# andi611/ZeroSpeech-TTS-without-T

Measured on AMD Instinct MI355X. Metric: mel-frames/sec (train_ae, seg_len=128, enc_size=1024), higher is better.
Workload: dtype bf16; 1 GPU; train_ae english hps seg_len=128 enc_size=1024 emb_size=1024 n_speakers=102 F=513, batch=256/GPU, dropout+Gumbel on, fwd+bwd+clip+Adam; global_batch=256, parallelism=dp1

## Files before the change

zerospeech-tts-without-t_amd/csrc/zs_gemm.hip:

```cpp
#include <stdlib.h>

#include <atomic>
#include <mutex>

#include "zs_common.h"

namespace {

constexpr int BM = 128, BN = 128, NT = 256;
constexpr int ROWB = 128;
constexpr int PITCH = 144;
constexpr int TILE_BYTES = BM * PITCH;

__device__ const uint4 zs_zero_line[8] = {};

__device__ __forceinline__ int xcd_remap(int bid, int nwg) {
  const int q = nwg >> 3, r = nwg & 7, xcd = bid & 7;
  return (xcd < r ? xcd * (q + 1) : r * (q + 1) + (xcd - r) * q) + (bid >> 3);
}

__device__ __forceinline__ int conv_src_row(int gather, int pad_mode, int stride, int pad_left, int T_in, int t,
                                            int j, bool& ok) {
  if (gather == 0) {
    int s = t * stride + j - pad_left;
// ... 1224 lines not shown
__device__ __forceinline__ void wgrad_tile_store(const ZsGemmWgrad& p, unsigned char* smem, f32x16 (&acc)[2][2], bool do_bias,
                                                 const float (&bsum)[LPT][EPS], const int (&lrow)[LPT], const int (&lseg)[LPT],
                                                 int split, int nsplit, int co0, int ci0, int tap, int cout_r, int cin_r, int wm, int wn,
                                                 int lane, int tid) {
  if (do_bias) {
    float* red = reinterpret_cast<float*>(smem);
#pragma unroll
    for (int i = 0; i < LPT; ++i)
#pragma unroll
      for (int e = 0; e < EPS; ++e) red[lrow[i] * 128 + lseg[i] * EPS + e] = bsum[i][e];
    __syncthreads();
    if (tid < 128) {
      float t = 0.f;
#pragma unroll 8
      for (int r = 0; r < WK; ++r) t += red[r * 128 + tid];
      float* bslab = (float*)p.workspace + (int64_t)nsplit * cout_r * p.taps * cin_r + (int64_t)split * cout_r;
      bslab[co0 + tid] = t;
    }
  }
  float* slab = (float*)p.workspace + (int64_t)split * cout_r * p.taps * cin_r;
  float* sC = reinterpret_cast<float*>(smem);
  __syncthreads();
#pragma unroll
  for (int mi = 0; mi < 2; ++mi)
#pragma unroll
    for (int ni = 0; ni < 2; ++ni)
#pragma unroll
      for (int r = 0; r < 16; ++r) {
        const int row = wm * 64 + mi * 32 + (r & 3) + 8 * (r >> 2) + 4 * (lane >> 5);
        const int col = wn * 64 + ni * 32 + (lane & 31);
        sC[row * CPITCH + col] = acc[mi][ni][r];
      }
  __syncthreads();
  const int cg = tid & 15, rr0 = tid >> 4;
#pragma unroll 1
  for (int it = 0; it < 8; ++it) {
    const int row = rr0 + 16 * it;
    const float4 x0 = *reinterpret_cast<const float4*>(sC + row * CPITCH + cg * 8);
    const float4 x1 = *reinterpret_cast<const float4*>(sC + row * CPITCH + cg * 8 + 4);
    float* d = slab + ((int64_t)(co0 + row) * p.taps + tap) * cin_r + ci0 + cg * 8;
    *reinterpret_cast<float4*>(d) = x0;
    *reinterpret_cast<float4*>(d + 4) = x1;
  }
}

template <typename T>
__global__ __launch_bounds__(NT, 2) void gemm_wgrad_kernel(const ZsGemmWgrad p, int ci_tiles, int rows_per_split,
                                                          int cout_r, int cin_r) {
  const Geom2 g2 = make_geom2(p.w_in, p.w_out, p.taps_h, p.T_in);
  constexpr int EPS = 16 / (int)sizeof(T);
  constexpr int SPR = 128 / EPS;
  constexpr int LPT = (WK * SPR) / NT;
  constexpr int PITCHW = WFrag<T>::PITCHW;
  constexpr int TILEW = WK * PITCHW;
  extern __shared__ __attribute__((aligned(16))) unsigned char smem[];
  unsigned char* sY = smem;
  unsigned char* sX = smem + 2 * TILEW;

  const int tid = threadIdx.x, lane = tid & 63, wave = tid >> 6;
  const int wm = wave >> 1, wn = wave & 1;
  const int per_co = p.taps * ci_tiles;
  const int tiles = ((cout_r / 128) * per_co);
  const int vid = xcd_remap(blockIdx.x, gridDim.x);
  const int split = vid / tiles, tile = vid - split * tiles;
  const int cot = tile / per_co;
  const int rem = tile - cot * per_co;
  const int tap = rem / ci_tiles, cit = rem - tap * ci_tiles;
  const int co0 = cot * 128, ci0 = cit * 128;
  const int M = p.B * p.T_out;
  const int nsplit = gridDim.x / tiles;
  const int mbeg = split * rows_per_split;
  const int mend = min(M, mbeg + rows_per_split);
  const T* __restrict__ dY = (const T*)p.dY;
  const T* __restrict__ X = (const T*)p.X;

  int lrow[LPT], lseg[LPT], lb[LPT], lt[LPT];
#pragma unroll
  for (int i = 0; i < LPT; ++i) {
    const int idx = tid + NT * i;
    lrow[i] = idx / SPR; lseg[i] = idx - lrow[i] * SPR;
    const int m = mbeg + lrow[i];
    lb[i] = m / p.T_out; lt[i] = m - lb[i] * p.T_out;
  }
  uint4 vy[LPT], vx[LPT];
  const bool do_bias = (p.db != nullptr) && tap == 0 && cit == 0;
  float bsum[LPT][EPS];
#pragma unroll
  for (int i = 0; i < LPT; ++i)
#pragma unroll
    for (int e = 0; e < EPS; ++e) bsum[i][e] = 0.f;
  auto gload = [&](int mb) {
#pragma unroll
    for (int i = 0; i < LPT; ++i) {
      const int m = mb + lrow[i];
      const int cy = co0 + lseg[i] * EPS, cx = ci0 + lseg[i] * EPS;
      vy[i] = make_uint4(0, 0, 0, 0); vx[i] = make_uint4(0, 0, 0, 0);
      if (m < mend) {
        if (cy < p.y_cols) vy[i] = *reinterpret_cast<const uint4*>(dY + (int64_t)m * p.ldy + cy);
        bool ok; const int s = conv_src_row_g(0, p.pad_mode, p.stride, p.pad_left, p.T_in, lt[i], tap, ok, g2);
        if (ok && cx < p.x_cols)
          vx[i] = *reinterpret_cast<const uint4*>(X + (int64_t)lb[i] * p.x_batch_stride + (int64_t)s * p.ldx + cx);
      }
      lt[i] += WK;
      while (lt[i] >= p.T_out) { lt[i] -= p.T_out; ++lb[i]; }
    }
  };
  auto swrite = [&](int buf) {
#pragma unroll
    for (int i = 0; i < LPT; ++i) {
      *reinterpret_cast<uint4*>(sY + buf * TILEW + lrow[i] * PITCHW + lseg[i] * 16) = vy[i];
      *reinterpret_cast<uint4*>(sX + buf * TILEW + lrow[i] * PITCHW + lseg[i] * 16) = vx[i];
      if (do_bias) {
        const uint32_t w4[4] = {vy[i].x, vy[i].y, vy[i].z, vy[i].w};
        if constexpr (sizeof(T) == 4) {
#pragma unroll
          for (int e = 0; e < 4; ++e) bsum[i][e] += __uint_as_float(w4[e]);
        } else {
#pragma unroll
          for (int e = 0; e < 4; ++e) {
            bsum[i][2 * e] += __uint_as_float(w4[e] << 16);
            bsum[i][2 * e + 1] += __uint_as_float(w4[e] & 0xffff0000u);
          }
        }
      }
    }
  };

  f32x16 acc[2][2];
#pragma unroll
  for (int i = 0; i < 2; ++i)
#pragma unroll
    for (int j = 0; j < 2; ++j)
#pragma unroll
      for (int r = 0; r < 16; ++r) acc[i][j][r] = 0.f;

  const int nchunks = (mend - mbeg + WK - 1) / WK;
  if (nchunks > 0) {
    gload(mbeg);
    swrite(0);
  }
  __syncthreads();
  for (int c = 0; c < nchunks; ++c) {
    const int buf = c & 1;
    if (c + 1 < nchunks) gload(mbeg + (c + 1) * WK);
    WFrag<T>::chunk(sY + buf * TILEW, sX + buf * TILEW, wm, wn, lane, acc);
    if (c + 1 < nchunks) swrite(buf ^ 1);
    __syncthreads();
  }

  wgrad_tile_store<LPT, EPS>(p, smem, acc, do_bias, bsum, lrow, lseg, split, nsplit, co0, ci0, tap, cout_r, cin_r, wm, wn, lane, tid);
}

#define ZS_DSRT(dst, addr, off) asm volatile("ds_read_b64_tr_b16 %0, %1 offset:" #off : "=v"(dst) : "v"(addr))
#define ZS_WP_READ_A(base)                                                                        \
  ZS_DSRT(ya00, sa0, base + 0);    ZS_DSRT(yb00, sa0, base + 512);  ZS_DSRT(ya01, sa1, base + 0);    ZS_DSRT(yb01, sa1, base + 512);  \
  ZS_DSRT(ya10, sa0, base + 2048); ZS_DSRT(yb10, sa0, base + 2560); ZS_DSRT(ya11, sa1, base + 2048); ZS_DSRT(yb11, sa1, base + 2560); \
  ZS_DSRT(ya20, sa0, base + 4096); ZS_DSRT(yb20, sa0, base + 4608); ZS_DSRT(ya21, sa1, base + 4096); ZS_DSRT(yb21, sa1, base + 4608); \
  ZS_DSRT(ya30, sa0, base + 6144); ZS_DSRT(yb30, sa0, base + 6656); ZS_DSRT(ya31, sa1, base + 6144); ZS_DSRT(yb31, sa1, base + 6656);
#define ZS_WP_READ_B(x, sbx)                                                                      \
  ZS_DSRT(x##a0, sbx, 0);    ZS_DSRT(x##b0, sbx, 512);  ZS_DSRT(x##a1, sbx, 2048); ZS_DSRT(x##b1, sbx, 2560); \
  ZS_DSRT(x##a2, sbx, 4096); ZS_DSRT(x##b2, sbx, 4608); ZS_DSRT(x##a3, sbx, 6144); ZS_DSRT(x##b3, sbx, 6656);
#define ZS_WP_MMA(alo, ahi, blo, bhi, c)                                                          \
  c = __builtin_amdgcn_mfma_f32_32x32x16_bf16(__builtin_bit_cast(bf16x8, make_uint4(alo.x, alo.y, ahi.x, ahi.y)), \
                                               __builtin_bit_cast(bf16x8, make_uint4(blo.x, blo.y, bhi.x, bhi.y)), c, 0, 0, 0)
#define ZS_WP_DMA(cond, src, dst)                                                                 \
  __builtin_amdgcn_sched_barrier(0);                                                              \
  if (cond) __builtin_amdgcn_global_load_lds((gptr_t)(src), (lptr_t)(dst), 16, 0, 0);             \
  __builtin_amdgcn_sched_barrier(0);
#define ZS_WP_QUAD(c0, c1, x, cond, src0, dst0, src1, dst1)                                        \
  __builtin_amdgcn_s_setprio(1);                                                                  \
  ZS_WP_MMA(ya00, yb00, x##a0, x##b0, c0); ZS_WP_MMA(ya01, yb01, x##a0, x##b0, c1);               \
  ZS_WP_DMA(cond, src0, dst0)                                                                     \
  ZS_WP_MMA(ya10, yb10, x##a1, x##b1, c0); ZS_WP_MMA(ya11, yb11, x##a1, x##b1, c1); ZS_WP_MMA(ya20, yb20, x##a2, x##b2, c0); \
  ZS_WP_DMA(cond, src1, dst1)                                                                     \
  ZS_WP_MMA(ya21, yb21, x##a2, x##b2, c1); ZS_WP_MMA(ya30, yb30, x##a3, x##b3, c0); ZS_WP_MMA(ya31, yb31, x##a3, x##b3, c1); \
  __builtin_amdgcn_s_setprio(0);

__global__ __launch_bounds__(PNT, 2) void gemm_wgrad_p8_kernel(const ZsGemmWgrad p, int ci_tiles, int rows_per_split,
                                                              int cout_r, int cin_r) {
  const Geom2 g2 = make_geom2(p.w_in, p.w_out, p.taps_h, p.T_in);
  typedef bf16_t T;
  extern __shared__ __attribute__((aligned(16))) unsigned char smem[];
  typedef __attribute__((address_space(1))) const void* gptr_t;
  typedef __attribute__((address_space(3))) void* lptr_t;
  const int tid = threadIdx.x, lane = tid & 63, wave = __builtin_amdgcn_readfirstlane(tid >> 6);
  const int wr = wave >> 2, wc = wave & 3;
  const int per_co = p.taps * ci_tiles;
  const int tiles = (cout_r / 256) * per_co;
  const int vid = xcd_remap(blockIdx.x, gridDim.x);
  const int split = vid / tiles, tile = vid - split * tiles;
  const int cot = tile / per_co;
  const int rem = tile - cot * per_co;
  const int tap = rem / ci_tiles, cit = rem - tap * ci_tiles;
  const int co0 = cot * 256, ci0 = cit * 256;
  const int M = p.B * p.T_out;
  const int nsplit = gridDim.x / tiles;
  const int mbeg = split * rows_per_split;
  const int mend = min(M, mbeg + rows_per_split);
  const int nk = (mend - mbeg + 63) / 64;
  const T* __restrict__ dY = (const T*)p.dY;
  const T* __restrict__ X = (const T*)p.X;
  const T* zline = reinterpret_cast<const T*>(zs_zero_line);

  const int lrow = lane >> 3, slot = lane & 7;
  const int k0 = (wave & 3) * 16 + lrow, k1 = k0 + 8;
  const int cbl = wave >> 2;
  const int sg0 = slot ^ (((k0 >> 1) & 1) << 2), sg1 = slot ^ (((k1 >> 1) & 1) << 2);
  const int yc0 = co0 + cbl * 64 + sg0 * 8, yc1 = co0 + cbl * 64 + sg1 * 8;
  const int xc0 = ci0 + cbl * 64 + sg0 * 8, xc1 = ci0 + cbl * 64 + sg1 * 8;
  auto y_ptr = [&](int m, int col) -> const T* {
    return (m < mend && col < p.y_cols) ? dY + (int64_t)m * p.ldy + col : zline;
  };
  auto x_row = [&](int m, bool& ok) -> const T* {
    ok = false;
    if (m >= mend) return zline;
    const int b = m / p.T_out, t = m - b * p.T_out;
    const int srow = conv_src_row_g(0, p.pad_mode, p.stride, p.pad_left, p.T_in, t, tap, ok, g2);
    return X + (int64_t)b * p.x_batch_stride + (int64_t)srow * p.ldx;
  };

  unsigned char* const ldsA = smem + wave * 2048;
  unsigned char* const ldsB = smem + 32768 + wave * 2048;

  f32x16 c000, c001, c010, c011, c100, c101, c110, c111;
#pragma unroll
  for (int r = 0; r < 16; ++r) { c000[r] = 0.f; c001[r] = 0.f; c010[r] = 0.f; c011[r] = 0.f; c100[r] = 0.f; c101[r] = 0.f; c110[r] = 0.f; c111[r] = 0.f; }

  const int gi = lane >> 4, q = (lane >> 2) & 3, pp = lane & 3;
  const int sw = ((q >> 1) & 1) << 2;
  const int segl = 2 * (gi & 1) + (pp >> 1);
  const unsigned lds0 = (unsigned)(uintptr_t)(__attribute__((address_space(3))) unsigned char*)smem;
  const unsigned rowoff = (unsigned)((8 * (gi >> 1) + q) * 128 + (pp & 1) * 8);
  const unsigned a_l0 = lds0 + (unsigned)(wr * 2 * 64 * 128) + rowoff + (unsigned)(((0 + segl) ^ sw) * 16);
  const unsigned a_l1 = lds0 + (unsigned)(wr * 2 * 64 * 128) + rowoff + (unsigned)(((4 + segl) ^ sw) * 16);
  const unsigned b_l0 = lds0 + 32768u + (unsigned)(wc * 64 * 128) + rowoff + (unsigned)(((0 + segl) ^ sw) * 16);
  const unsigned b_l1 = lds0 + 32768u + (unsigned)(wc * 64 * 128) + rowoff + (unsigned)(((4 + segl) ^ sw) * 16);
  const int grp1 = wr;

  const bool do_bias = (p.db != nullptr) && tap == 0 && cit == 0;
  const int tg = tid & 255, seg16 = tg & 15, kr0 = tg >> 4;
  const unsigned bias_addr = lds0 + (unsigned)(((wr * 2 + (seg16 >> 3)) * 64 + kr0) * 128 + (((seg16 & 7) ^ (((kr0 >> 1) & 1) << 2)) * 16));
  float bsum[8];
#pragma unroll
  for (int e = 0; e < 8; ++e) bsum[e] = 0.f;

  {
    __builtin_amdgcn_global_load_lds((gptr_t)y_ptr(mbeg + k0, yc0), (lptr_t)(ldsA), 16, 0, 0);
    __builtin_amdgcn_global_load_lds((gptr_t)y_ptr(mbeg + k1, yc1), (lptr_t)(ldsA + 1024), 16, 0, 0);
    __builtin_amdgcn_global_load_lds((gptr_t)y_ptr(mbeg + k0, yc0 + 128), (lptr_t)(ldsA + 16384), 16, 0, 0);
    __builtin_amdgcn_global_load_lds((gptr_t)y_ptr(mbeg + k1, yc1 + 128), (lptr_t)(ldsA + 16384 + 1024), 16, 0, 0);
#pragma unroll
    for (int tt = 0; tt < 2; ++tt) {
      if (tt < nk) {
        bool ok0, ok1;
        const T* r0 = x_row(mbeg + tt * 64 + k0, ok0);
        const T* r1 = x_row(mbeg + tt * 64 + k1, ok1);
        unsigned char* d = ldsB + tt * PSTAGE;
        __builtin_amdgcn_global_load_lds((gptr_t)((ok0 && xc0 < p.x_cols) ? r0 + xc0 : zline), (lptr_t)(d), 16, 0, 0);
        __builtin_amdgcn_global_load_lds((gptr_t)((ok1 && xc1 < p.x_cols) ? r1 + xc1 : zline), (lptr_t)(d + 1024), 16, 0, 0);
        __builtin_amdgcn_global_load_lds((gptr_t)((ok0 && xc0 + 128 < p.x_cols) ? r0 + xc0 + 128 : zline), (lptr_t)(d + 16384), 16, 0, 0);
        __builtin_amdgcn_global_load_lds((gptr_t)((ok1 && xc1 + 128 < p.x_cols) ? r1 + xc1 + 128 : zline), (lptr_t)(d + 16384 + 1024), 16, 0, 0);
      }
    }
    if (nk > 1) asm volatile("s_waitcnt vmcnt(4)" ::: "memory");
    else asm volatile("s_waitcnt vmcnt(0)" ::: "memory");
  }
  __builtin_amdgcn_s_barrier();
  if (grp1) __builtin_amdgcn_s_barrier();

  uint2 ya00, yb00, ya01, yb01, ya10, yb10, ya11, yb11, ya20, yb20, ya21, yb21, ya30, yb30, ya31, yb31;
  uint2 f0a0, f0b0, f0a1, f0b1, f0a2, f0b2, f0a3, f0b3;
  uint2 f1a0, f1b0, f1a1, f1b1, f1a2, f1b2, f1a3, f1b3;
  for (int kt = 0; kt < nk; ++kt) {
    const int st = kt & 1;
    const unsigned so = (unsigned)(st * PSTAGE);
    const unsigned sa0 = a_l0 + so, sa1 = a_l1 + so, sb0 = b_l0 + so, sb1 = b_l1 + so;
    const bool has_a = kt + 1 < nk, has_b = kt + 2 < nk;
    unsigned char* const dA = ldsA + (st ^ 1) * PSTAGE;
    unsigned char* const dB = ldsB + st * PSTAGE;
    const int ma = mbeg + (kt + 1) * 64, mb = mbeg + (kt + 2) * 64;
    ZS_WP_READ_A(0)
    ZS_WP_READ_B(f0, sb0)
    const T* s0 = y_ptr(ma + k0, yc0);
    const T* s1 = y_ptr(ma + k1, yc1);
    asm volatile("s_waitcnt lgkmcnt(0)" ::: "memory");
    __builtin_amdgcn_s_barrier();
    __builtin_amdgcn_sched_barrier(0);
    ZS_WP_QUAD(c000, c001, f0, has_a, s0, dA, s1, dA + 1024)
    __builtin_amdgcn_s_barrier();
    __builtin_amdgcn_sched_barrier(0);
    ZS_WP_READ_B(f1, sb1)
    s0 = y_ptr(ma + k0, yc0 + 128);
    s1 = y_ptr(ma + k1, yc1 + 128);
    if (do_bias) {
      u32x4_t v0, v1, v2, v3;
      const unsigned ba = bias_addr + so;
      ZS_DSR(v0, ba, 0); ZS_DSR(v1, ba, 2048); ZS_DSR(v2, ba, 4096); ZS_DSR(v3, ba, 6144);
      asm volatile("s_waitcnt lgkmcnt(0)" ::: "memory");
      const unsigned w[16] = {v0.x, v0.y, v0.z, v0.w, v1.x, v1.y, v1.z, v1.w, v2.x, v2.y, v2.z, v2.w, v3.x, v3.y, v3.z, v3.w};
#pragma unroll
      for (int i = 0; i < 16; ++i) {
        bsum[2 * (i & 3)] += __uint_as_float(w[i] << 16);
        bsum[2 * (i & 3) + 1] += __uint_as_float(w[i] & 0xffff0000u);
      }
    }
    asm volatile("s_waitcnt lgkmcnt(0)" ::: "memory");
    __builtin_amdgcn_s_barrier();
    __builtin_amdgcn_sched_barrier(0);
    ZS_WP_QUAD(c010, c011, f1, has_a, s0, dA + 16384, s1, dA + 16384 + 1024)
    __builtin_amdgcn_s_barrier();
    __builtin_amdgcn_sched_barrier(0);
    ZS_WP_READ_A(8192)
    bool ok0, ok1;
    const T* r0 = x_row(mb + k0, ok0);
    const T* r1 = x_row(mb + k1, ok1);
    s0 = (ok0 && xc0 < p.x_cols) ? r0 + xc0 : zline;
    s1 = (ok1 && xc1 < p.x_cols) ? r1 + xc1 : zline;
    asm volatile("s_waitcnt lgkmcnt(0)" ::: "memory");
    __builtin_amdgcn_s_barrier();
    __builtin_amdgcn_sched_barrier(0);
    ZS_WP_QUAD(c110, c111, f1, has_b, s0, dB, s1, dB + 1024)
    __builtin_amdgcn_s_barrier();
    __builtin_amdgcn_sched_barrier(0);
    s0 = (ok0 && xc0 + 128 < p.x_cols) ? r0 + xc0 + 128 : zline;
    s1 = (ok1 && xc1 + 128 < p.x_cols) ? r1 + xc1 + 128 : zline;
    if (grp1) {
      if (has_b) asm volatile("s_waitcnt vmcnt(2)" ::: "memory");
      else asm volatile("s_waitcnt vmcnt(0)" ::: "memory");
    }
    __builtin_amdgcn_s_barrier();
    __builtin_amdgcn_sched_barrier(0);
    ZS_WP_QUAD(c100, c101, f0, has_b, s0, dB + 16384, s1, dB + 16384 + 1024)
    if (!grp1) {
      if (has_b) asm volatile("s_waitcnt vmcnt(4)" ::: "memory");
      else asm volatile("s_waitcnt vmcnt(0)" ::: "memory");
    }
    __builtin_amdgcn_s_barrier();
    __builtin_amdgcn_sched_barrier(0);
  }
  if (!grp1) __builtin_amdgcn_s_barrier();
  asm volatile("s_waitcnt vmcnt(0)" ::: "memory");
  __syncthreads();

  if (do_bias) {
    float* red = reinterpret_cast<float*>(smem);
#pragma unroll
    for (int e = 0; e < 8; ++e) red[(wr * 16 + kr0) * 128 + seg16 * 8 + e] = bsum[e];
    __syncthreads();
    if (tid < 256) {
      float t = 0.f;
#pragma unroll
      for (int r = 0; r < 16; ++r) t += red[((tid >> 7) * 16 + r) * 128 + (tid & 127)];
      float* bslab = (float*)p.workspace + (int64_t)nsplit * cout_r * p.taps * cin_r + (int64_t)split * cout_r;
      bslab[co0 + tid] = t;
    }
    __syncthreads();
  }
  float* slab = (float*)p.workspace + (int64_t)split * cout_r * p.taps * cin_r;
  float* sC = reinterpret_cast<float*>(smem);
#pragma unroll 1
  for (int h = 0; h < 2; ++h) {
    if ((wc >> 1) == h) {
      const int cb = (wc & 1) * 64 + (lane & 31);
      const int rbase = wr * 128 + 4 * (lane >> 5);
#pragma unroll
      for (int r = 0; r < 16; ++r) {
        const int ro = (r & 3) + 8 * (r >> 2);
        sC[(rbase + ro) * CPITCH + cb] = c000[r];            sC[(rbase + 32 + ro) * CPITCH + cb] = c001[r];
        sC[(rbase + ro) * CPITCH + cb + 32] = c010[r];       sC[(rbase + 32 + ro) * CPITCH + cb + 32] = c011[r];
        sC[(rbase + 64 + ro) * CPITCH + cb] = c100[r];       sC[(rbase + 96 + ro) * CPITCH + cb] = c101[r];
        sC[(rbase + 64 + ro) * CPITCH + cb + 32] = c110[r];  sC[(rbase + 96 + ro) * CPITCH + cb + 32] = c111[r];
      }
    }
    __syncthreads();
    const int cg = tid & 15, rr0 = tid >> 4;
#pragma unroll 1
    for (int it = 0; it < 8; ++it) {
      const int row = rr0 + 32 * it;
      const float4 x0 = *reinterpret_cast<const float4*>(sC + row * CPITCH + cg * 8);
      const float4 x1 = *reinterpret_cast<const float4*>(sC + row * CPITCH + cg * 8 + 4);
      float* d = slab + ((int64_t)(co0 + row) * p.taps + tap) * cin_r + ci0 + h * 128 + cg * 8;
      *reinterpret_cast<float4*>(d) = x0;
      *reinterpret_cast<float4*>(d + 4) = x1;
    }
    __syncthreads();
  }
}

constexpr int WDSTAGE = 2 * 2 * 64 * 128;
constexpr int WD_LDS = (2 * WDSTAGE > EPI_LDS_BYTES) ? 2 * WDSTAGE : EPI_LDS_BYTES;

__global__ __launch_bounds__(NT, 2) void gemm_wgrad_dma_kernel(const ZsGemmWgrad p, int ci_tiles, int rows_per_split, int cout_r,
                                                              int cin_r) {
  const Geom2 g2 = make_geom2(p.w_in, p.w_out, p.taps_h, p.T_in);
  typedef bf16_t T;
  typedef __attribute__((address_space(1))) const void* gptr_t;
  typedef __attribute__((address_space(3))) void* lptr_t;
  extern __shared__ __attribute__((aligned(16))) unsigned char smem[];
  const int tid = threadIdx.x, lane = tid & 63, wave = __builtin_amdgcn_readfirstlane(tid >> 6);
  const int wm = wave >> 1, wn = wave & 1;
  const int per_co = p.taps * ci_tiles;
  const int tiles = (cout_r / 128) * per_co;
  const int vid = xcd_remap(blockIdx.x, gridDim.x);
  const int split = vid / tiles, tile = vid - split * tiles;
  const int cot = tile / per_co;
  const int rem = tile - cot * per_co;
  const int tap = rem / ci_tiles, cit = rem - tap * ci_tiles;
  const int co0 = cot * 128, ci0 = cit * 128;
  const int M = p.B * p.T_out;
  const int nsplit = gridDim.x / tiles;
  const int mbeg = split * rows_per_split;
  const int mend = min(M, mbeg + rows_per_split);
  const int nk = (mend - mbeg + 63) / 64;
  const T* __restrict__ dY = (const T*)p.dY;
  const T* __restrict__ X = (const T*)p.X;
  const T* zline = reinterpret_cast<const T*>(zs_zero_line);

  const int lrow8 = lane >> 3, slot = lane & 7;
  const int k0 = wave * 16 + lrow8, k1 = k0 + 8;
  const int sg0 = slot ^ (((k0 >> 1) & 1) << 2), sg1 = slot ^ (((k1 >> 1) & 1) << 2);
  auto dma = [&](int kt, int st) {
    unsigned char* const dy = smem + st * WDSTAGE + wave * 2048;
    unsigned char* const dx = dy + 16384;
#pragma unroll
    for (int h = 0; h < 2; ++h) {
      const int m = mbeg + kt * 64 + (h ? k1 : k0);
      const int sg = h ? sg1 : sg0;
      const bool in = m < mend;
      bool ok = false;
      const T* xr = zline;
      if (in) {
        const int b = m / p.T_out, t = m - b * p.T_out;
        const int srow = conv_src_row_g(0, p.pad_mode, p.stride, p.pad_left, p.T_in, t, tap, ok, g2);
        xr = X + (int64_t)b * p.x_batch_stride + (int64_t)srow * p.ldx;
      }
      const T* yr = dY + (int64_t)m * p.ldy;
#pragma unroll
      for (int cb = 0; cb < 2; ++cb) {
        const int cy = co0 + cb * 64 + sg * 8, cx = ci0 + cb * 64 + sg * 8;
        __builtin_amdgcn_global_load_lds((gptr_t)((in && cy < p.y_cols) ? yr + cy : zline), (lptr_t)(dy + cb * 8192 + h * 1024), 16, 0, 0);
        __builtin_amdgcn_global_load_lds((gptr_t)((ok && cx < p.x_cols) ? xr + cx : zline), (lptr_t)(dx + cb * 8192 + h * 1024), 16, 0, 0);
      }
    }
  };

  const int gi = lane >> 4, q = (lane >> 2) & 3, pp = lane & 3;
  const int sw = ((q >> 1) & 1) << 2;
  const int segl = 2 * (gi & 1) + (pp >> 1);
  const unsigned lds0 = (unsigned)(uintptr_t)(__attribute__((address_space(3))) unsigned char*)smem;
  const unsigned rowoff = (unsigned)((8 * (gi >> 1) + q) * 128 + (pp & 1) * 8);
  const unsigned a_l0 = lds0 + (unsigned)(wm * 8192) + rowoff + (unsigned)(((0 + segl) ^ sw) * 16);
  const unsigned a_l1 = lds0 + (unsigned)(wm * 8192) + rowoff + (unsigned)(((4 + segl) ^ sw) * 16);
  const unsigned b_l0 = lds0 + 16384u + (unsigned)(wn * 8192) + rowoff + (unsigned)(((0 + segl) ^ sw) * 16);
  const unsigned b_l1 = lds0 + 16384u + (unsigned)(wn * 8192) + rowoff + (unsigned)(((4 + segl) ^ sw) * 16);

  const bool do_bias = (p.db != nullptr) && tap == 0 && cit == 0;
  int lrow[2], lseg[2];
#pragma unroll
  for (int i = 0; i < 2; ++i) { lrow[i] = (tid >> 4) + 16 * i; lseg[i] = tid & 15; }
  const int bcb = (tid & 15) >> 3, bg8 = tid & 7;
  const int boff = bcb * 8192 + (tid >> 4) * 128 + ((bg8 ^ ((((tid >> 4) >> 1) & 1) << 2)) * 16);
  float bsum[2][8];
#pragma unroll
  for (int i = 0; i < 2; ++i)
#pragma unroll
    for (int e = 0; e < 8; ++e) bsum[i][e] = 0.f;

  f32x16 acc[2][2];
#pragma unroll
  for (int i = 0; i < 2; ++i)
#pragma unroll
    for (int j = 0; j < 2; ++j)
#pragma unroll
      for (int r = 0; r < 16; ++r) acc[i][j][r] = 0.f;

  if (nk > 0) dma(0, 0);
  uint2 y0a0, y0b0, y0a1, y0b1, y0a2, y0b2, y0a3, y0b3, y1a0, y1b0, y1a1, y1b1, y1a2, y1b2, y1a3, y1b3;
  uint2 x0a0, x0b0, x0a1, x0b1, x0a2, x0b2, x0a3, x0b3, x1a0, x1b0, x1a1, x1b1, x1a2, x1b2, x1a3, x1b3;
  for (int kt = 0; kt < nk; ++kt) {
    const int st = kt & 1;
    asm volatile("s_waitcnt vmcnt(0)" ::: "memory");
    __syncthreads();
    if (kt + 1 < nk) dma(kt + 1, st ^ 1);
    const unsigned so = (unsigned)(st * WDSTAGE);
    const unsigned sa0 = a_l0 + so, sa1 = a_l1 + so, sb0 = b_l0 + so, sb1 = b_l1 + so;
    ZS_WP_READ_B(y0, sa0)
    ZS_WP_READ_B(y1, sa1)
    ZS_WP_READ_B(x0, sb0)
    ZS_WP_READ_B(x1, sb1)
    if (do_bias) {
      const unsigned char* by = smem + st * WDSTAGE + boff;
      const uint4 v0 = *reinterpret_cast<const uint4*>(by), v1 = *reinterpret_cast<const uint4*>(by + 16 * 128);
      const uint4 v2 = *reinterpret_cast<const uint4*>(by + 32 * 128), v3 = *reinterpret_cast<const uint4*>(by + 48 * 128);
      const uint32_t w[4][4] = {{v0.x, v0.y, v0.z, v0.w}, {v1.x, v1.y, v1.z, v1.w}, {v2.x, v2.y, v2.z, v2.w}, {v3.x, v3.y, v3.z, v3.w}};
#pragma unroll
      for (int c = 0; c < 4; ++c)
#pragma unroll
        for (int e = 0; e < 4; ++e) {
          bsum[c & 1][2 * e] += __uint_as_float(w[c][e] << 16);
          bsum[c & 1][2 * e + 1] += __uint_as_float(w[c][e] & 0xffff0000u);
        }
    }
    asm volatile("s_waitcnt lgkmcnt(0)" ::: "memory");
    __builtin_amdgcn_sched_barrier(0);
#define ZS_WD_KS(ks)                                                                                                    \
    ZS_WP_MMA(y0a##ks, y0b##ks, x0a##ks, x0b##ks, acc[0][0]); ZS_WP_MMA(y0a##ks, y0b##ks, x1a##ks, x1b##ks, acc[0][1]); \
    ZS_WP_MMA(y1a##ks, y1b##ks, x0a##ks, x0b##ks, acc[1][0]); ZS_WP_MMA(y1a##ks, y1b##ks, x1a##ks, x1b##ks, acc[1][1]);
    ZS_WD_KS(0) ZS_WD_KS(1) ZS_WD_KS(2) ZS_WD_KS(3)
#undef ZS_WD_KS
  }
  asm volatile("s_waitcnt vmcnt(0)" ::: "memory");
  __syncthreads();
  wgrad_tile_store<2, 8>(p, smem, acc, do_bias, bsum, lrow, lseg, split, nsplit, co0, ci0, tap, cout_r, cin_r, wm, wn, lane, tid);
}

__device__ __forceinline__ float4 wgrad_sum_splits(const float* ws, int splits, int64_t sstride) {
  float4 acc = make_float4(0.f, 0.f, 0.f, 0.f);
  int k = 0;
  for (; k + 8 <= splits; k += 8) {
    float4 v[8];
#pragma unroll
    for (int u = 0; u < 8; ++u) v[u] = *reinterpret_cast<const float4*>(ws + (int64_t)(k + u) * sstride);
#pragma unroll
    for (int u = 0; u < 8; ++u) { acc.x += v[u].x; acc.y += v[u].y; acc.z += v[u].z; acc.w += v[u].w; }
  }
  for (; k < splits; ++k) {
    const float4 v = *reinterpret_cast<const float4*>(ws + (int64_t)k * sstride);
    acc.x += v.x; acc.y += v.y; acc.z += v.z; acc.w += v.w;
  }
  return acc;
}

__device__ __forceinline__ int wgrad_co_perm(const ZsGemmWgrad& p, int co) {
  return p.co_split2 ? ((co & 1) * (p.Cout >> 1) + (co >> 1)) : co;
}

__device__ __forceinline__ void wgrad_reduce_bias(const ZsGemmWgrad& p, int splits, int cout_r, int64_t sstride, int bblk) {
  const int co = bblk * 256 + (int)threadIdx.x;
  if (co >= p.Cout) return;
// ... 131 lines not shown
                       reinterpret_cast<const void*>(gemm_wgrad_p8_kernel)};
  for (const void* f : big) (void)hipFuncSetAttribute(f, hipFuncAttributeMaxDynamicSharedMemorySize, P8_LDS);
  const void* ring[] = {reinterpret_cast<const void*>(gemm_conv_ring_kernel<float, 0>), reinterpret_cast<const void*>(gemm_conv_ring_kernel<bf16_t, 0>),
                        reinterpret_cast<const void*>(gemm_conv_ring_kernel<float, 1>), reinterpret_cast<const void*>(gemm_conv_ring_kernel<bf16_t, 1>)};
  for (const void* f : ring) (void)hipFuncSetAttribute(f, hipFuncAttributeMaxDynamicSharedMemorySize, RING_LDS);
}

}

extern "C" int zs_gemm_conv(const ZsGemmConv* p, void* stream) {
  ZS_REQUIRE(p && p->A && p->W && (p->out || p->out2), "zs_gemm_conv: null operand");
  ZS_REQUIRE(p->dtype == ZS_F32 || p->dtype == ZS_BF16, "zs_gemm_conv: bad dtype %d", p->dtype);
  const int es = p->dtype == ZS_F32 ? 4 : 2;
  const int kc = 128 / es;
  ZS_REQUIRE(p->B > 0 && p->T_in > 0 && p->T_out > 0 && p->N > 0 && p->taps > 0 && p->stride > 0, "zs_gemm_conv: bad sizes");
  ZS_REQUIRE(p->cin_pad > 0 && p->cin_pad % kc == 0, "zs_gemm_conv: cin_pad %d must be a multiple of %d (one 128-byte chunk)", p->cin_pad, kc);
  ZS_REQUIRE(p->ldw >= (int64_t)p->taps * p->cin_pad && (p->ldw * es) % 16 == 0, "zs_gemm_conv: ldw %lld < taps*cin_pad",
             (long long)p->ldw);
  ZS_REQUIRE(p->n_pad % 128 == 0 && p->n_pad >= p->N, "zs_gemm_conv: n_pad %d must be a multiple of 128 >= N %d", p->n_pad, p->N);
  ZS_REQUIRE(aligned16(p->A) && aligned16(p->W) && (p->lda * es) % 16 == 0 && (p->a_batch_stride * es) % 16 == 0 &&
                 (p->a_gstride * es) % 16 == 0 && (p->w_gstride * es) % 16 == 0,
             "zs_gemm_conv: operands must be 16-byte aligned (A=%p lda=%lld)", p->A, (long long)p->lda);
  if (p->w_in > 0) {
    ZS_REQUIRE((int64_t)p->T_out * p->w_out < (1ll << 32), "zs_gemm_conv: 2-D image too large (T_out %d x w_out %d)", p->T_out, p->w_out);
    ZS_REQUIRE(p->w_out > 0 && p->taps_h > 0 && p->taps % p->taps_h == 0 && p->T_in % p->w_in == 0 && p->T_out % p->w_out == 0 && !p->lengths,
               "zs_gemm_conv: 2-D geometry (w_in %d, w_out %d, taps_h %d, taps %d, T_in %d, T_out %d)", p->w_in, p->w_out, p->taps_h, p->taps,
               p->T_in, p->T_out);
    if (p->gather == 0 && p->pad_mode == ZS_PAD_REFLECT) {
      const int h_in = p->T_in / p->w_in, h_out = p->T_out / p->w_out, taps_w = p->taps / p->taps_h;
      const int pr_h = (h_out - 1) * p->stride + p->taps_h - 1 - p->pad_left - (h_in - 1);
      const int pr_w = (p->w_out - 1) * p->stride + taps_w - 1 - p->pad_left - (p->w_in - 1);
      ZS_REQUIRE(p->pad_left < h_in && pr_h < h_in && p->pad_left < p->w_in && pr_w < p->w_in,
                 "zs_gemm_conv: Padding size should be less than the corresponding input dimension (2-D: pad %d, H %d, W %d)", p->pad_left, h_in, p->w_in);
    }
  } else if (p->gather == 0 && p->pad_mode == ZS_PAD_REFLECT) {
    const int pad_r = (p->T_out - 1) * p->stride + p->taps - 1 - p->pad_left - (p->T_in - 1);
    ZS_REQUIRE(p->pad_left < p->T_in && pad_r < p->T_in,
               "zs_gemm_conv: Padding size should be less than the corresponding input dimension (pad %d/%d, T %d)",
               p->pad_left, pad_r, p->T_in);
  }
  if (p->store_mode == ZS_STORE_SPLIT2 || (p->out2 && p->store_mode2 == ZS_STORE_SPLIT2))
    ZS_REQUIRE(p->N % 2 == 0, "zs_gemm_conv: SPLIT2 needs even N");
  ZS_REQUIRE(!(p->pre_vec || p->vec2) || p->vec_idx, "zs_gemm_conv: vec_idx missing");
  ZS_REQUIRE(!p->colsum || (128 % p->T_out == 0 && p->colsum_col0 >= 0 && p->colsum_col0 < p->N && !p->bias && !p->pre_vec &&
                            p->act == ZS_ACT_NONE && p->groups <= 1),
             "zs_gemm_conv: colsum needs T_out (%d) to divide 128, 0 <= colsum_col0 < N and no bias / pre_vec / activation / groups", p->T_out);
  ZS_REQUIRE(!p->lengths || (p->gather == 0 && p->B < 65536 && p->T_in < 32768 && p->pad_right >= 0 && p->colsum == nullptr),
             "zs_gemm_conv: lengths (ragged batch) needs gather 0, B < 65536, T_in < 32768, pad_right >= 0 and no colsum");
  const int groups = p->groups > 0 ? p->groups : 1;
  const int64_t M = (int64_t)p->B * p->T_out;
  const int64_t tiles = ((M + BM - 1) / BM) * ((p->N + BN - 1) / BN);
  ZS_REQUIRE(tiles < (1ll << 31), "zs_gemm_conv: grid too large");
  dim3 grid((unsigned)tiles, 1, (unsigned)groups);
  hipStream_t s = (hipStream_t)stream;
  std::call_once(g_lds_attr_once, set_lds_attrs);
  const int use_dma = g_use_dma.get(), use_ring = g_use_ring.get(), use_p8 = g_use_p8.get(), use_pp = g_use_pp.get();
  const int64_t ring_tiles = ((M + RBM - 1) / RBM) * ((p->N + BN - 1) / BN);
  const int64_t p8_tiles = ((M + PBM - 1) / PBM) * ((p->N + PBN - 1) / PBN);
  if (use_dma && use_p8 && p->n_pad % PBN == 0 && p8_tiles >= g_p8_min_tiles.get() && p8_tiles < (1ll << 31)) {
    dim3 pgrid((unsigned)p8_tiles, 1, (unsigned)groups);
    if (p->dtype == ZS_F32) hipLaunchKernelGGL(gemm_conv_p8m16_kernel<float>, pgrid, dim3(PNT), P8_LDS, s, *p);
    else hipLaunchKernelGGL(gemm_conv_p8m16_kernel<bf16_t>, pgrid, dim3(PNT), P8_LDS, s, *p);
  } else if (use_dma && use_ring && ring_tiles >= g_ring_min_tiles.get() && ring_tiles < (1ll << 31)) {
    dim3 rgrid((unsigned)ring_tiles, 1, (unsigned)groups);
    if (use_pp) {
      if (p->dtype == ZS_F32) hipLaunchKernelGGL((gemm_conv_ring_kernel<float, 1>), rgrid, dim3(RNT), RING_LDS, s, *p);
      else hipLaunchKernelGGL((gemm_conv_ring_kernel<bf16_t, 1>), rgrid, dim3(RNT), RING_LDS, s, *p);
    } else {
      if (p->dtype == ZS_F32) hipLaunchKernelGGL((gemm_conv_ring_kernel<float, 0>), rgrid, dim3(RNT), RING_LDS, s, *p);
      else hipLaunchKernelGGL((gemm_conv_ring_kernel<bf16_t, 0>), rgrid, dim3(RNT), RING_LDS, s, *p);
    }
  } else if (use_dma) {
    const int64_t tiles64 = ((M + 63) / 64) * ((p->N + BN - 1) / BN);
    if (g_dma64.get() && tiles * 2 <= g_dma64_max_tiles.get() && tiles64 < (1ll << 31) && (p->colsum == nullptr || 64 % p->T_out == 0)) {
      dim3 g64((unsigned)tiles64, 1, (unsigned)groups);
      const size_t lds = (2 * 64 * 128 + 2 * DTILE > EPI_LDS_BYTES / 2) ? 2 * 64 * 128 + 2 * DTILE : EPI_LDS_BYTES / 2;
      if (p->dtype == ZS_F32) hipLaunchKernelGGL((gemm_conv_dma_kernel<float, 64>), g64, dim3(NT), lds, s, *p);
      else hipLaunchKernelGGL((gemm_conv_dma_kernel<bf16_t, 64>), g64, dim3(NT), lds, s, *p);
      return zs_check_launch("zs_gemm_conv");
    }
    const size_t lds = (4 * DTILE > EPI_LDS_BYTES) ? 4 * DTILE : EPI_LDS_BYTES;
    if (p->dtype == ZS_F32) hipLaunchKernelGGL((gemm_conv_dma_kernel<float, 128>), grid, dim3(NT), lds, s, *p);
    else hipLaunchKernelGGL((gemm_conv_dma_kernel<bf16_t, 128>), grid, dim3(NT), lds, s, *p);
  } else {
    const size_t lds = 4 * TILE_BYTES;
    if (p->dtype == ZS_F32) hipLaunchKernelGGL(gemm_conv_kernel<float>, grid, dim3(NT), lds, s, *p);
    else hipLaunchKernelGGL(gemm_conv_kernel<bf16_t>, grid, dim3(NT), lds, s, *p);
  }
  return zs_check_launch("zs_gemm_conv");
}

extern "C" size_t zs_gemm_wgrad_workspace_bytes(const ZsGemmWgrad* p) {
  if (!p) return 0;
  const WgradPlan w = wgrad_plan(p);
  return (size_t)w.splits * ((size_t)w.cout_r * p->taps * w.cin_r + w.cout_r) * sizeof(float);
}

extern "C" int zs_gemm_wgrad(const ZsGemmWgrad* p, void* stream) {
  ZS_REQUIRE(p && p->dY && p->X && p->dW && p->workspace, "zs_gemm_wgrad: null operand");
  ZS_REQUIRE(aligned16(p->workspace), "zs_gemm_wgrad: workspace must be 16-byte aligned");
  ZS_REQUIRE(p->dtype == ZS_F32 || p->dtype == ZS_BF16, "zs_gemm_wgrad: bad dtype");
  const int es = p->dtype == ZS_F32 ? 4 : 2;
  ZS_REQUIRE(p->B > 0 && p->T_in > 0 && p->T_out > 0 && p->Cout > 0 && p->Cin > 0 && p->taps > 0 && p->stride > 0,
             "zs_gemm_wgrad: bad sizes");
  ZS_REQUIRE(aligned16(p->dY) && aligned16(p->X) && (p->ldy * es) % 16 == 0 && (p->ldx * es) % 16 == 0 &&
                 (p->x_batch_stride * es) % 16 == 0 && (p->y_cols * es) % 16 == 0 && (p->x_cols * es) % 16 == 0,
             "zs_gemm_wgrad: operands must be 16-byte aligned");
  ZS_REQUIRE(p->y_cols <= p->ldy && p->x_cols <= p->ldx && p->Cout <= p->y_cols && p->Cin <= p->x_cols, "zs_gemm_wgrad: column bounds");
  ZS_REQUIRE(!p->co_split2 || p->Cout % 2 == 0, "zs_gemm_wgrad: SPLIT2 needs even Cout");
  ZS_REQUIRE(p->w_in == 0 || (p->w_in > 0 && p->w_out > 0 && p->taps_h > 0 && p->taps % p->taps_h == 0 && p->T_in % p->w_in == 0 &&
                              p->T_out % p->w_out == 0 && (int64_t)p->T_out * p->w_out < (1ll << 32)),
             "zs_gemm_wgrad: 2-D geometry (w_in %d, w_out %d, taps_h %d, taps %d, T_in %d, T_out %d)", p->w_in, p->w_out, p->taps_h, p->taps,
             p->T_in, p->T_out);
  const WgradPlan w = wgrad_plan(p);
  const int splits = w.splits, co_tiles = w.co_tiles, ci_tiles = w.ci_tiles, cout_r = w.cout_r, cin_r = w.cin_r;
  const int rows_per_split = w.rows_per_split;
  const size_t need = (size_t)splits * ((size_t)cout_r * p->taps * cin_r + cout_r) * sizeof(float);
  if (p->workspace_bytes < need) {
    zs_set_error("zs_gemm_wgrad: workspace %zu < %zu bytes", p->workspace_bytes, need);
    return ZS_EWORKSPACE;
  }
  hipStream_t s = (hipStream_t)stream;
  ZS_REQUIRE((int64_t)co_tiles * p->taps * ci_tiles * splits < (1ll << 31), "zs_gemm_wgrad: grid too large");
  dim3 grid((unsigned)(co_tiles * p->taps * ci_tiles * splits), 1, 1);
  std::call_once(g_lds_attr_once, set_lds_attrs);
  if (w.p8) {
    hipLaunchKernelGGL(gemm_wgrad_p8_kernel, grid, dim3(PNT), P8_LDS, s, *p, ci_tiles, rows_per_split, cout_r, cin_r);
  } else if (p->dtype == ZS_F32) {
    const size_t lds = (4 * WK * WFrag<float>::PITCHW > EPI_LDS_BYTES) ? 4 * WK * WFrag<float>::PITCHW : EPI_LDS_BYTES;
    hipLaunchKernelGGL(gemm_wgrad_kernel<float>, grid, dim3(NT), lds, s, *p, ci_tiles, rows_per_split, cout_r, cin_r);
  } else if (w.dma) {
    hipLaunchKernelGGL(gemm_wgrad_dma_kernel, grid, dim3(NT), WD_LDS, s, *p, ci_tiles, rows_per_split, cout_r, cin_r);
  } else {
    const size_t lds = (4 * WK * WFrag<bf16_t>::PITCHW > EPI_LDS_BYTES) ? 4 * WK * WFrag<bf16_t>::PITCHW : EPI_LDS_BYTES;
    hipLaunchKernelGGL(gemm_wgrad_kernel<bf16_t>, grid, dim3(NT), lds, s, *p, ci_tiles, rows_per_split, cout_r, cin_r);
  }
  int rc = zs_check_launch("zs_gemm_wgrad");
  if (rc) return rc;
  const int nbias = p->db ? (p->Cout + 255) / 256 : 0;
  if (g_wgrad_reduce_taps.get() && p->taps > 1 && p->taps <= 256 && p->si == p->taps && p->sj == 1) {
    const int c4n = 256 / p->taps;
    const int nblk = (p->Cin + 4 * c4n - 1) / (4 * c4n);
    ZS_REQUIRE((int64_t)p->Cout * nblk + nbias < (1ll << 31), "zs_gemm_wgrad: reduce grid too large");
    const int nmain = p->Cout * nblk;
    hipLaunchKernelGGL(wgrad_reduce_taps_kernel, dim3((unsigned)(nmain + nbias)), dim3(256), 0, s, *p, splits, cout_r, cin_r, c4n, nblk, nmain);
  } else {
    const int64_t relems = (int64_t)p->Cout * p->taps * ((p->Cin + 3) / 4);
    const int64_t nmain = (relems + 255) / 256;
    ZS_REQUIRE(nmain + nbias < (1ll << 31), "zs_gemm_wgrad: reduce grid too large");
    hipLaunchKernelGGL(wgrad_reduce_kernel, dim3((unsigned)(nmain + nbias)), dim3(256), 0, s, *p, splits, cout_r, cin_r, (int)nmain);
  }
  return zs_check_launch("zs_gemm_wgrad.reduce");
}
```

Before: 2.978 million frames/s.

## Interleave LDS transpose reads with MFMAs and carry row pointers in wgrad p8 kernel

Splits the bulk A/B LDS transpose reads of the wgrad p8 kernel into per-k-slice groups and interleaves them with the MFMA sequence using partial lgkmcnt waits, so LDS latency hides behind matrix math. It also replaces per-iteration row-address recomputation (division and conv source row lookup) with incrementally advanced pointers, including a carried X-pointer path when the sequence length divides 128. Column-bound checks are hoisted out of the loop. Optional cycle-counter profiling is added behind a compile flag. The hand-tuned waitcnt counts are fragile and register pressure rises.

Result: faster. 3.056 million frames/s, median of 6 (+2.6%).

```diff
diff --git a/zerospeech-tts-without-t_amd/csrc/zs_gemm.hip b/zerospeech-tts-without-t_amd/csrc/zs_gemm.hip
--- a/zerospeech-tts-without-t_amd/csrc/zs_gemm.hip
+++ b/zerospeech-tts-without-t_amd/csrc/zs_gemm.hip
@@ -1400,11 +1400,18 @@
 }
 
 #define ZS_DSRT(dst, addr, off) asm volatile("ds_read_b64_tr_b16 %0, %1 offset:" #off : "=v"(dst) : "v"(addr))
-#define ZS_WP_READ_A(base)                                                                        \
-  ZS_DSRT(ya00, sa0, base + 0);    ZS_DSRT(yb00, sa0, base + 512);  ZS_DSRT(ya01, sa1, base + 0);    ZS_DSRT(yb01, sa1, base + 512);  \
-  ZS_DSRT(ya10, sa0, base + 2048); ZS_DSRT(yb10, sa0, base + 2560); ZS_DSRT(ya11, sa1, base + 2048); ZS_DSRT(yb11, sa1, base + 2560); \
-  ZS_DSRT(ya20, sa0, base + 4096); ZS_DSRT(yb20, sa0, base + 4608); ZS_DSRT(ya21, sa1, base + 4096); ZS_DSRT(yb21, sa1, base + 4608); \
-  ZS_DSRT(ya30, sa0, base + 6144); ZS_DSRT(yb30, sa0, base + 6656); ZS_DSRT(ya31, sa1, base + 6144); ZS_DSRT(yb31, sa1, base + 6656);
+#define ZS_WP_RA(ks, o0, o1)                                                                      \
+  __builtin_amdgcn_sched_barrier(0);                                                              \
+  ZS_DSRT(ya##ks##0, sa0, o0); ZS_DSRT(yb##ks##0, sa0, o1); ZS_DSRT(ya##ks##1, sa1, o0); ZS_DSRT(yb##ks##1, sa1, o1); \
+  __builtin_amdgcn_sched_barrier(0);
+#define ZS_WP_RB(x, ks, sbx, o0, o1)                                                              \
+  __builtin_amdgcn_sched_barrier(0);                                                              \
+  ZS_DSRT(x##a##ks, sbx, o0); ZS_DSRT(x##b##ks, sbx, o1);                                         \
+  __builtin_amdgcn_sched_barrier(0);
+#define ZS_WP_WAIT(n)                                                                             \
+  __builtin_amdgcn_sched_barrier(0);                                                              \
+  asm volatile("s_waitcnt lgkmcnt(" #n ")" ::: "memory");                                         \
+  __builtin_amdgcn_sched_barrier(0);
 #define ZS_WP_READ_B(x, sbx)                                                                      \
   ZS_DSRT(x##a0, sbx, 0);    ZS_DSRT(x##b0, sbx, 512);  ZS_DSRT(x##a1, sbx, 2048); ZS_DSRT(x##b1, sbx, 2560); \
   ZS_DSRT(x##a2, sbx, 4096); ZS_DSRT(x##b2, sbx, 4608); ZS_DSRT(x##a3, sbx, 6144); ZS_DSRT(x##b3, sbx, 6656);
@@ -1423,6 +1430,15 @@
   ZS_WP_DMA(cond, src1, dst1)                                                                     \
   ZS_WP_MMA(ya21, yb21, x##a2, x##b2, c1); ZS_WP_MMA(ya30, yb30, x##a3, x##b3, c0); ZS_WP_MMA(ya31, yb31, x##a3, x##b3, c1); \
   __builtin_amdgcn_s_setprio(0);
+
+#ifdef ZS_WGP8_PROFILE
+__device__ unsigned long long zs_wgp8_prof[2][24];
+#define ZS_WPT(k) { __builtin_amdgcn_sched_barrier(0); const long long pt1_ = __builtin_readcyclecounter(); pc[k] += pt1_ - pt0; pt0 = pt1_; \
+                    __builtin_amdgcn_sched_barrier(0); }
+#else
+#define ZS_WPT(k)
+#endif
+__device__ __forceinline__ bool wgrad_p8_carried(const ZsGemmWgrad& p) { return p.w_in == 0 && p.stride == 1 && (128 % p.T_out) == 0; }
 
 __global__ __launch_bounds__(PNT, 2) void gemm_wgrad_p8_kernel(const ZsGemmWgrad p, int ci_tiles, int rows_per_split,
                                                               int cout_r, int cin_r) {
@@ -1459,14 +1475,24 @@
   auto y_ptr = [&](int m, int col) -> const T* {
     return (m < mend && col < p.y_cols) ? dY + (int64_t)m * p.ldy + col : zline;
   };
-  auto x_row = [&](int m, bool& ok) -> const T* {
-    ok = false;
-    if (m >= mend) return zline;
+  auto x_src = [&](int m, bool& ok) -> const T* {
     const int b = m / p.T_out, t = m - b * p.T_out;
     const int srow = conv_src_row_g(0, p.pad_mode, p.stride, p.pad_left, p.T_in, t, tap, ok, g2);
     return X + (int64_t)b * p.x_batch_stride + (int64_t)srow * p.ldx;
   };
-
+  auto x_row = [&](int m, bool& ok) -> const T* {
+    ok = false;
+    if (m >= mend) return zline;
+    return x_src(m, ok);
+  };
+  const bool ycv0 = yc0 < p.y_cols, ycv1 = yc1 < p.y_cols, ycv0h = yc0 + 128 < p.y_cols, ycv1h = yc1 + 128 < p.y_cols;
+  const bool xcv0 = xc0 < p.x_cols, xcv1 = xc1 < p.x_cols, xcv0h = xc0 + 128 < p.x_cols, xcv1h = xc1 + 128 < p.x_cols;
+
+#ifdef ZS_WGP8_PROFILE
+  long long pc[19], pt0 = __builtin_readcyclecounter();
+#pragma unroll
+  for (int i = 0; i < 19; ++i) pc[i] = 0;
+#endif
   unsigned char* const ldsA = smem + wave * 2048;
   unsigned char* const ldsB = smem + 32768 + wave * 2048;
 
@@ -1515,6 +1541,19 @@
   }
   __builtin_amdgcn_s_barrier();
   if (grp1) __builtin_amdgcn_s_barrier();
+  ZS_WPT(0)
+
+  const int64_t ystep = (int64_t)64 * p.ldy;
+  const T* py0 = dY + (int64_t)(mbeg + 64 + k0) * p.ldy + yc0;
+  const T* py1 = dY + (int64_t)(mbeg + 64 + k1) * p.ldy + yc1;
+  const bool carried = wgrad_p8_carried(p);
+  const int64_t xstep = carried ? (int64_t)(128 / p.T_out) * p.x_batch_stride : 0;
+  const T *px0c = zline, *px0n = zline, *px1c = zline, *px1n = zline;
+  bool xo0c = false, xo0n = false, xo1c = false, xo1n = false;
+  if (carried) {
+    px0c = x_src(mbeg + 128 + k0, xo0c) + xc0; px0n = x_src(mbeg + 192 + k0, xo0n) + xc0;
+    px1c = x_src(mbeg + 128 + k1, xo1c) + xc1; px1n = x_src(mbeg + 192 + k1, xo1n) + xc1;
+  }
 
   uint2 ya00, yb00, ya01, yb01, ya10, yb10, ya11, yb11, ya20, yb20, ya21, yb21, ya30, yb30, ya31, yb31;
   uint2 f0a0, f0b0, f0a1, f0b1, f0a2, f0b2, f0a3, f0b3;
@@ -1527,19 +1566,38 @@
     unsigned char* const dA = ldsA + (st ^ 1) * PSTAGE;
     unsigned char* const dB = ldsB + st * PSTAGE;
     const int ma = mbeg + (kt + 1) * 64, mb = mbeg + (kt + 2) * 64;
-    ZS_WP_READ_A(0)
-    ZS_WP_READ_B(f0, sb0)
-    const T* s0 = y_ptr(ma + k0, yc0);
-    const T* s1 = y_ptr(ma + k1, yc1);
-    asm volatile("s_waitcnt lgkmcnt(0)" ::: "memory");
+    ZS_WP_RB(f0, 0, sb0, 0, 512) ZS_WP_RA(0, 0, 512) ZS_WP_RB(f0, 1, sb0, 2048, 2560) ZS_WP_RA(1, 2048, 2560)
+    const bool yv0 = ma + k0 < mend, yv1 = ma + k1 < mend;
+    const T* s0 = (yv0 && ycv0) ? py0 : zline;
+    const T* s1 = (yv1 && ycv1) ? py1 : zline;
+    ZS_WP_WAIT(6)
+    ZS_WPT(1)
     __builtin_amdgcn_s_barrier();
     __builtin_amdgcn_sched_barrier(0);
-    ZS_WP_QUAD(c000, c001, f0, has_a, s0, dA, s1, dA + 1024)
+    ZS_WPT(2)
+    __builtin_amdgcn_s_setprio(1);
+    ZS_WP_MMA(ya00, yb00, f0a0, f0b0, c000); ZS_WP_RB(f0, 2, sb0, 4096, 4608)
+    ZS_WP_MMA(ya01, yb01, f0a0, f0b0, c001); ZS_WP_RA(2, 4096, 4608)
+    ZS_WP_DMA(has_a, s0, dA)
+    ZS_WP_WAIT(6)
+    ZS_WP_MMA(ya10, yb10, f0a1, f0b1, c000); ZS_WP_RB(f0, 3, sb0, 6144, 6656)
+    ZS_WP_MMA(ya11, yb11, f0a1, f0b1, c001); ZS_WP_RA(3, 6144, 6656)
+    ZS_WP_WAIT(6)
+    ZS_WP_MMA(ya20, yb20, f0a2, f0b2, c000);
+    ZS_WP_DMA(has_a, s1, dA + 1024)
+    ZS_WP_RB(f1, 0, sb1, 0, 512) ZS_WP_RB(f1, 1, sb1, 2048, 2560)
+    ZS_WP_MMA(ya21, yb21, f0a2, f0b2, c001);
+    ZS_WP_RB(f1, 2, sb1, 4096, 4608) ZS_WP_RB(f1, 3, sb1, 6144, 6656)
+    ZS_WP_WAIT(8)
+    ZS_WP_MMA(ya30, yb30, f0a3, f0b3, c000); ZS_WP_MMA(ya31, yb31, f0a3, f0b3, c001);
+    __builtin_amdgcn_s_setprio(0);
+    ZS_WPT(3)
     __builtin_amdgcn_s_barrier();
     __builtin_amdgcn_sched_barrier(0);
-    ZS_WP_READ_B(f1, sb1)
-    s0 = y_ptr(ma + k0, yc0 + 128);
-    s1 = y_ptr(ma + k1, yc1 + 128);
+    ZS_WPT(4)
+    s0 = (yv0 && ycv0h) ? py0 + 128 : zline;
+    s1 = (yv1 && ycv1h) ? py1 + 128 : zline;
+    py0 += ystep; py1 += ystep;
     if (do_bias) {
       u32x4_t v0, v1, v2, v3;
       const unsigned ba = bias_addr + so;
@@ -1552,39 +1610,80 @@
         bsum[2 * (i & 3) + 1] += __uint_as_float(w[i] & 0xffff0000u);
       }
     }
-    asm volatile("s_waitcnt lgkmcnt(0)" ::: "memory");
+    ZS_WP_WAIT(0)
+    ZS_WPT(5)
     __builtin_amdgcn_s_barrier();
     __builtin_amdgcn_sched_barrier(0);
-    ZS_WP_QUAD(c010, c011, f1, has_a, s0, dA + 16384, s1, dA + 16384 + 1024)
+    ZS_WPT(6)
+    __builtin_amdgcn_s_setprio(1);
+    ZS_WP_MMA(ya00, yb00, f1a0, f1b0, c010); ZS_WP_MMA(ya01, yb01, f1a0, f1b0, c011);
+    ZS_WP_DMA(has_a, s0, dA + 16384)
+    ZS_WP_MMA(ya10, yb10, f1a1, f1b1, c010); ZS_WP_MMA(ya11, yb11, f1a1, f1b1, c011);
+    ZS_WP_RA(0, 8192, 8704)
+    ZS_WP_MMA(ya20, yb20, f1a2, f1b2, c010);
+    ZS_WP_DMA(has_a, s1, dA + 16384 + 1024)
+    ZS_WP_MMA(ya21, yb21, f1a2, f1b2, c011);
+    ZS_WP_RA(1, 10240, 10752)
+    ZS_WP_MMA(ya30, yb30, f1a3, f1b3, c010); ZS_WP_MMA(ya31, yb31, f1a3, f1b3, c011);
+    ZS_WP_RA(2, 12288, 12800)
+    __builtin_amdgcn_s_setprio(0);
+    ZS_WPT(7)
     __builtin_amdgcn_s_barrier();
     __builtin_amdgcn_sched_barrier(0);
-    ZS_WP_READ_A(8192)
+    ZS_WPT(8)
     bool ok0, ok1;
-    const T* r0 = x_row(mb + k0, ok0);
-    const T* r1 = x_row(mb + k1, ok1);
-    s0 = (ok0 && xc0 < p.x_cols) ? r0 + xc0 : zline;
-    s1 = (ok1 && xc1 < p.x_cols) ? r1 + xc1 : zline;
-    asm volatile("s_waitcnt lgkmcnt(0)" ::: "memory");
+    const T *r0, *r1;
+    if (carried) {
+      ok0 = xo0c && (mb + k0 < mend); ok1 = xo1c && (mb + k1 < mend);
+      r0 = px0c; r1 = px1c;
+      const T* n0 = px0c + xstep; const T* n1 = px1c + xstep;
+      px0c = px0n; px1c = px1n; px0n = n0; px1n = n1;
+      const bool t0 = xo0c, t1 = xo1c;
+      xo0c = xo0n; xo1c = xo1n; xo0n = t0; xo1n = t1;
+    } else {
+      r0 = x_row(mb + k0, ok0) + xc0;
+      r1 = x_row(mb + k1, ok1) + xc1;
+    }
+    s0 = (ok0 && xcv0) ? r0 : zline;
+    s1 = (ok1 && xcv1) ? r1 : zline;
+    ZS_WP_RA(3, 14336, 14848)
+    ZS_WP_WAIT(4)
+    ZS_WPT(9)
     __builtin_amdgcn_s_barrier();
     __builtin_amdgcn_sched_barrier(0);
-    ZS_WP_QUAD(c110, c111, f1, has_b, s0, dB, s1, dB + 1024)
+    ZS_WPT(10)
+    __builtin_amdgcn_s_setprio(1);
+    ZS_WP_MMA(ya00, yb00, f1a0, f1b0, c110); ZS_WP_MMA(ya01, yb01, f1a0, f1b0, c111);
+    ZS_WP_DMA(has_b, s0, dB)
+    ZS_WP_MMA(ya10, yb10, f1a1, f1b1, c110); ZS_WP_MMA(ya11, yb11, f1a1, f1b1, c111); ZS_WP_MMA(ya20, yb20, f1a2, f1b2, c110);
+    ZS_WP_DMA(has_b, s1, dB + 1024)
+    ZS_WP_MMA(ya21, yb21, f1a2, f1b2, c111);
+    ZS_WP_WAIT(0)
+    ZS_WP_MMA(ya30, yb30, f1a3, f1b3, c110); ZS_WP_MMA(ya31, yb31, f1a3, f1b3, c111);
+    __builtin_amdgcn_s_setprio(0);
+    ZS_WPT(11)
     __builtin_amdgcn_s_barrier();
     __builtin_amdgcn_sched_barrier(0);
-    s0 = (ok0 && xc0 + 128 < p.x_cols) ? r0 + xc0 + 128 : zline;
-    s1 = (ok1 && xc1 + 128 < p.x_cols) ? r1 + xc1 + 128 : zline;
+    ZS_WPT(12)
+    s0 = (ok0 && xcv0h) ? r0 + 128 : zline;
+    s1 = (ok1 && xcv1h) ? r1 + 128 : zline;
     if (grp1) {
       if (has_b) asm volatile("s_waitcnt vmcnt(2)" ::: "memory");
       else asm volatile("s_waitcnt vmcnt(0)" ::: "memory");
     }
+    ZS_WPT(13)
     __builtin_amdgcn_s_barrier();
     __builtin_amdgcn_sched_barrier(0);
+    ZS_WPT(14)
     ZS_WP_QUAD(c100, c101, f0, has_b, s0, dB + 16384, s1, dB + 16384 + 1024)
+    ZS_WPT(15)
     if (!grp1) {
       if (has_b) asm volatile("s_waitcnt vmcnt(4)" ::: "memory");
       else asm volatile("s_waitcnt vmcnt(0)" ::: "memory");
     }
     __builtin_amdgcn_s_barrier();
     __builtin_amdgcn_sched_barrier(0);
+    ZS_WPT(16)
   }
   if (!grp1) __builtin_amdgcn_s_barrier();
   asm volatile("s_waitcnt vmcnt(0)" ::: "memory");
@@ -1606,6 +1705,7 @@
   }
   float* slab = (float*)p.workspace + (int64_t)split * cout_r * p.taps * cin_r;
   float* sC = reinterpret_cast<float*>(smem);
+  ZS_WPT(17)
 #pragma unroll 1
   for (int h = 0; h < 2; ++h) {
     if ((wc >> 1) == h) {
@@ -1633,6 +1733,15 @@
     }
     __syncthreads();
   }
+#ifdef ZS_WGP8_PROFILE
+  ZS_WPT(18)
+  if (lane == 0 && (wave & 3) == 0) {
+#pragma unroll
+    for (int i = 0; i < 19; ++i) atomicAdd(&zs_wgp8_prof[wr][i], (unsigned long long)pc[i]);
+    atomicAdd(&zs_wgp8_prof[wr][19], (unsigned long long)nk);
+    atomicAdd(&zs_wgp8_prof[wr][20], 1ull);
+  }
+#endif
 }
 
 constexpr int WDSTAGE = 2 * 2 * 64 * 128;
@@ -2070,3 +2179,15 @@
   }
   return zs_check_launch("zs_gemm_wgrad.reduce");
 }
+
+#ifdef ZS_WGP8_PROFILE
+extern "C" int zs_wgp8_profile_read(unsigned long long* out, int reset) {
+  if (hipDeviceSynchronize() != hipSuccess) return 1;
+  if (out && hipMemcpyFromSymbol(out, HIP_SYMBOL(zs_wgp8_prof), sizeof(unsigned long long) * 48) != hipSuccess) return 1;
+  if (reset) {
+    unsigned long long z[48] = {0};
+    if (hipMemcpyToSymbol(HIP_SYMBOL(zs_wgp8_prof), z, sizeof(z)) != hipSuccess) return 1;
+  }
+  return 0;
+}
+#endif
```
